# gbordelon/fast_ray_tracer

Hardware: AMD Instinct MI355X
Metric: Mrays/s (primary+shadow+secondary) + wall-clock/frame, 1/2/4/8 GPU (higher is better)
Workload: dtype f64

## Files before the change

### fast_ray_tracer_amd/csrc/frt_engine.hip

```cpp
#include <hip/hip_runtime.h>
#include <hipcub/hipcub.hpp>

#include <algorithm>
#include <array>
#include <atomic>
#include <condition_variable>
#include <memory>
#include <mutex>
#include <cmath>
#include <cstdio>
#include <cstdlib>
#include <cstring>
#include <string>
#include <chrono>
#include <functional>
#include <thread>
#include <vector>

#include "frt_device.h"
#include "frt_jit.h"
#include "frt_shade.hpp"
#include "frt_shade32.hpp"
#include "frt_shadow.hpp"
#include "frt_jit_rt.hpp"
// ... 21 lines not shown
static_assert(sizeof(NodeRec) == 216, "NodeRec layout");

struct NodeCore {
    int32_t material, flags, parent, slot;
    double normalv[3], eyev[3];
    double over_d, rf;
};
struct NodeColors {
    double Ka[3], Kd[3], Ks[3], refl[3];
    double Ns;
};
static_assert(sizeof(NodeCore) == 80 && sizeof(NodeColors) == 104, "NodeCols layout");
enum NodeFlags : int32_t { kReflApplies = 1, kRefrApplies = 2, kMix = 4, kDissolve = 8, kReflSpawned = 16, kRefrSpawned = 32 };
enum : int32_t { kOwnColors = 64, kOwnD = 128 };

struct NodeCols {
    Cols<NodeCore> core;
    Cols<NodeColors> col;
    HeadCols head;
    int32_t root = 0;
    int32_t eye_cam = 0;
    static size_t bytes(int64_t cap) { return Cols<NodeCore>::bytes(cap) + Cols<NodeColors>::bytes(cap); }
    void set(uint64_t* base, int64_t cap) {
        core.w = base;
        core.cap = cap;
        col.w = base + (size_t)Cols<NodeCore>::kWords * cap;
        col.cap = cap;
    }
    __device__ __forceinline__ void store(int64_t i, const NodeRec& v, bool own_colors, bool own_d) const {
        NodeCore c;
        for (int k = 0; k < 3; ++k) {
            c.normalv[k] = v.normalv[k];
            c.eyev[k] = v.eyev[k];
        }
        c.material = v.material;
        c.parent = v.parent;
        c.slot = v.slot;
        c.flags = v.flags | (own_colors ? kOwnColors : 0) | (own_d ? kOwnD : 0);
        c.over_d = v.over_d;
        c.rf = v.rf;
        uint64_t t[10];
        __builtin_memcpy(t, &c, sizeof(c));
        const int64_t cap = core.cap;
        core.w[i] = t[0];
        if (!root) core.w[cap + i] = t[1];
#pragma unroll
        for (int f = 2; f < 5; ++f) core.w[f * cap + i] = t[f];
        if (!eye_cam) {
#pragma unroll
            for (int f = 5; f < 8; ++f) core.w[f * cap + i] = t[f];
        }
        if (own_d) core.w[8 * cap + i] = t[8];
        if (c.flags & kMix) core.w[9 * cap + i] = t[9];
        if (own_colors) {
            NodeColors o;
            for (int k = 0; k < 3; ++k) {
                o.Ka[k] = v.Ka[k];
                o.Kd[k] = v.Kd[k];
                o.Ks[k] = v.Ks[k];
                o.refl[k] = v.refl[k];
            }
            o.Ns = v.Ns;
            col.store(i, o);
        }
    }
    __device__ __forceinline__ void store_miss(int64_t i, int32_t parent, int32_t slot) const {
        core.w[i] = (uint64_t)(uint32_t)-1;
        if (!root) core.w[core.cap + i] = (uint64_t)(uint32_t)parent | ((uint64_t)(uint32_t)slot << 32);
    }
    __device__ __forceinline__ NodeRec load(int64_t i, const frt_material* __restrict__ mats) const {
        uint64_t t[10];
        const int64_t cap = core.cap;
        t[0] = core.w[i];
        t[1] = root ? (uint64_t)(uint32_t)-1 : core.w[cap + i];
#pragma unroll
        for (int f = 2; f < 5; ++f) t[f] = core.w[f * cap + i];
#pragma unroll
        for (int f = 5; f < 8; ++f) t[f] = eye_cam ? 0ull : core.w[f * cap + i];
        const int32_t mat = (int32_t)(uint32_t)t[0], fl = (int32_t)(t[0] >> 32);
        const double od = (fl & kOwnD) ? __longlong_as_double((long long)core.w[8 * cap + i])
                          : mat >= 0 ? 1.0 - mats[mat].Tr : 0.0;
        const double rf = (fl & kMix) ? __longlong_as_double((long long)core.w[9 * cap + i]) : 0.0;
        t[8] = (uint64_t)__double_as_longlong(od);
        t[9] = (uint64_t)__double_as_longlong(rf);
        NodeCore c;
        __builtin_memcpy(&c, t, sizeof(c));
        NodeRec v;
        head.over_point(i, v.over_point);
        for (int k = 0; k < 3; ++k) {
            v.normalv[k] = c.normalv[k];
            v.eyev[k] = c.eyev[k];
        }
        v.key = head.key != nullptr ? head.key[i] : 0ull;
        v.material = c.material;
        v.parent = c.parent;
        v.slot = c.slot;
        v.flags = c.flags;
        v.over_d = c.over_d;
        v.rf = c.rf;
        if (c.material < 0) {
            for (int k = 0; k < 3; ++k) v.Ka[k] = v.Kd[k] = v.Ks[k] = v.refl[k] = 0.0;
            v.Ns = 0.0;
        } else if (c.flags & kOwnColors) {
// ... 380 lines not shown
#define FRT_SHADE_FACTOR 1
#endif
#ifndef FRT_SHADE_ALG
#define FRT_SHADE_ALG 1
#endif
#ifndef FRT_SHADE_SKIP
#define FRT_SHADE_SKIP 1
#endif
#ifndef FRT_SHADE_FMA
#define FRT_SHADE_FMA 1
#endif
__device__ __forceinline__ double dot3_shade(const double* a, const double* b) {
    if (FRT_SHADE_FMA) return __builtin_fma(a[0], b[0], __builtin_fma(a[1], b[1], a[2] * b[2]));
    return dot3(a, b);
}
__device__ __forceinline__ void camera_eyev(const DevScene& S, const Batch& B, int64_t i, double* eyev) {
    Ray r;
    uint64_t key;
    unsigned ce = 0;
    camera_ray(S, B, i, r, key, ce);
    for (int k = 0; k < 3; ++k) eyev[k] = r.d[k] * -1.0;
}

__global__ void __launch_bounds__(kBlock) k_view_rays(DevScene S, Batch B, const frt_camera* __restrict__ cams,
                                                      int32_t nviews, int64_t view_pixels, int64_t n,
                                                      QueuedRay* __restrict__ q, unsigned* err) {
    const int64_t i = (int64_t)blockIdx.x * blockDim.x + threadIdx.x;
    if (i >= n) return;
    const int64_t pix = B.pixel_begin + i / B.spp;
    const int view = (int)min((int64_t)(nviews - 1), pix / view_pixels);
    Batch Bv = B;
    Bv.pixel_begin = pix - (int64_t)view * view_pixels - i / B.spp;
    unsigned e = 0;
    auto emit = [&](const frt_camera& cam) {
        DevScene Sv = S;
        Sv.cam = cam;
// ... 396 lines not shown
        }
    for (int k = 0; k < 3; ++k) {
        out[k] = sA[k];
        out[4 + k] = 0.0;
        out[8 + k] = 0.0;
    }
    out[3] = out[7] = out[11] = 0.0;
}

constexpr int kShadeSegs = 64;
static_assert(kShadeSegs == jit::kMixSegs, "k_shade_lit reads its slots with jit::mix_slot");
template <bool kLazy>
__global__ void __launch_bounds__(kBlock) k_shade(DevScene S, Batch B, NodeCols rec, int64_t n,
                                                  const int32_t* __restrict__ counts, Cols<Tri9> surface,
                                                  uint32_t* __restrict__ lit, unsigned* __restrict__ lcount,
                                                  uint32_t segcap) {
    const int64_t i = (int64_t)blockIdx.x * blockDim.x + threadIdx.x;
    bool heavy = false, mine = false;
    NodeRec nr{};
    if (i < n) {
        nr = rec.load(i, S.materials);
        if (!kLazy) nr.key = rec.key(S, B, i);
        mine = nr.material >= 0;
        heavy = mine && lit != nullptr && shade_heavy(S, counts, i);
    }
    if (!kLazy && mine && !heavy) {
        double out[12];
        if (rec.eye_cam) camera_eyev(S, B, i, nr.eyev);
        shade_node(S, B, nr, i, counts, out);
        tri_store(surface, i, out);
    }
    if (lit != nullptr) {
        const unsigned long long m = __ballot(heavy);
        if (m) {
            const int lane = threadIdx.x & 63;
            const int seg = (int)(blockIdx.x % kShadeSegs);
            unsigned base = 0;
            if (lane == 0) base = atomicAdd(lcount + seg * jit::kMixLine, (unsigned)__popcll(m));
            base = __shfl(base, 0, 64);
            const unsigned at = base + (unsigned)__popcll(m & ((1ull << lane) - 1));
            if (heavy) lit[(size_t)seg * segcap + at] = (uint32_t)i;
        }
    }
// ... 56 lines not shown
    nodes[m] = i;
}

struct LitStage {
    double over_point[3], normalv[3], eyev[3];
    uint64_t key;
    int32_t material, flags;
    uint32_t node;
    int32_t c0;
};
static_assert(sizeof(LitStage) == 96, "LitStage layout");

__global__ void __launch_bounds__(kBlock) k_lit_stage(DevScene S, Batch B, NodeCols rec, const int32_t* __restrict__ counts,
                                                      const uint32_t* __restrict__ lit, const unsigned* __restrict__ lcount,
                                                      uint32_t segcap, int sort_light, uint32_t* __restrict__ rows,
                                                      uint32_t* __restrict__ vals, LitStage* __restrict__ stage) {
    const uint32_t m = blockIdx.x * blockDim.x + threadIdx.x;
    const unsigned total = lit_total(lcount);
    if (blockIdx.x * blockDim.x + (threadIdx.x & ~63u) >= total) return;
    const size_t slot = jit::mix_slot(m < total ? m : 0u, lcount, segcap);
    if (m >= total) return;
    const uint32_t i = lit[slot];
    NodeRec nr = rec.load(i, S.materials);
    nr.key = rec.key(S, B, i);
    if (rec.eye_cam) camera_eyev(S, B, i, nr.eyev);
    LitStage r;
    for (int k = 0; k < 3; ++k) {
        r.over_point[k] = nr.over_point[k];
        r.normalv[k] = nr.normalv[k];
        r.eyev[k] = nr.eyev[k];
    }
    r.key = nr.key;
    r.material = nr.material;
    r.flags = nr.flags;
    r.node = i;
    r.c0 = S.num_lights == 1 ? counts[i] : -1;
    uint64_t w[12];
    __builtin_memcpy(w, &r, sizeof(r));
    uint64_t* dst = (uint64_t*)(stage + m);
#pragma unroll
    for (int k = 0; k < 12; ++k) dst[k] = w[k];
    rows[m] = (uint32_t)light_row(S.lights[sort_light], B.seed, nr.key, sort_light, 1);
    vals[m] = m;
}

#ifndef FRT_SHADE_WAVES
#define FRT_SHADE_WAVES 4
#endif
template <bool kRows, bool kFast32>
__device__ __forceinline__ void shade_lit_body(const DevScene& S, const Batch& B, const NodeCols& rec,
                                               const int32_t* __restrict__ counts, Cols<Tri9> surface,
                                               const uint32_t* __restrict__ lit,
                                               const unsigned* __restrict__ lcount, uint32_t segcap,
                                               const uint32_t* __restrict__ flat,
                                               const LitStage* __restrict__ stage, uint32_t* __restrict__ spos,
                                               const Light32& F) {
    const uint32_t m = blockIdx.x * blockDim.x + threadIdx.x;
    const int lane = threadIdx.x & 63;
    const unsigned c = lcount[lane * jit::kMixLine];
    unsigned incl = c;
#pragma unroll
    for (int o = 1; o < 64; o <<= 1) {
        const unsigned t = __shfl_up(incl, o, 64);
        if (lane >= o) incl += t;
    }
    const unsigned total = __shfl(incl, 63, 64);
    if (blockIdx.x * blockDim.x + (threadIdx.x & ~63u) >= total) return;
    int64_t i = 0;
    NodeRec nr{};
    int32_t c0 = -1;
    const bool staged = kRows && stage != nullptr;
// ... 15 lines not shown
        nr.material = r.material;
        nr.flags = r.flags;
        c0 = r.c0;
        i = (int64_t)r.node;
    } else {
        if (flat != nullptr) {
            if (m >= total) return;
            i = (int64_t)flat[m];
        } else {
            const size_t slot = jit::mix_slot(m < total ? m : 0u, lcount, segcap);
            if (m >= total) return;
            i = (int64_t)lit[slot];
        }
        nr = rec.load(i, S.materials);
        nr.key = rec.key(S, B, i);
        if (rec.eye_cam) camera_eyev(S, B, i, nr.eyev);
    }
    if (staged) {
        if (nr.flags & kOwnColors) {
            const NodeColors o = rec.col.load(i);
            for (int k = 0; k < 3; ++k) {
                nr.Ka[k] = o.Ka[k];
                nr.Kd[k] = o.Kd[k];
                nr.Ks[k] = o.Ks[k];
            }
            nr.Ns = o.Ns;
        } else {
            const frt_material& M = S.materials[nr.material];
            for (int k = 0; k < 3; ++k) {
                nr.Ka[k] = M.Ka[k];
                nr.Kd[k] = M.Kd[k];
// ... 22 lines not shown
            dst[3 + k] = (uint64_t)__double_as_longlong(out[4 + k]);
            dst[6 + k] = (uint64_t)__double_as_longlong(out[8 + k]);
        }
        spos[i] = m;
        return;
    }
    tri_store(surface, i, out);
}

template <bool kRows>
__global__ void __launch_bounds__(kBlock) __attribute__((amdgpu_waves_per_eu(FRT_SHADE_WAVES, 8))) k_shade_lit(DevScene S, Batch B, NodeCols rec,
                                                      const int32_t* __restrict__ counts, Cols<Tri9> surface,
                                                      const uint32_t* __restrict__ lit,
                                                      const unsigned* __restrict__ lcount, uint32_t segcap,
                                                      const uint32_t* __restrict__ flat,
                                                      const LitStage* __restrict__ stage, uint32_t* __restrict__ spos) {
    shade_lit_body<kRows, false>(S, B, rec, counts, surface, lit, lcount, segcap, flat, stage, spos, Light32{});
}

template <bool kRows>
__global__ void __launch_bounds__(kBlock) k_shade_lit32(DevScene S, Batch B, NodeCols rec,
                                                        const int32_t* __restrict__ counts, Cols<Tri9> surface,
                                                        const uint32_t* __restrict__ lit,
                                                        const unsigned* __restrict__ lcount, uint32_t segcap,
                                                        const uint32_t* __restrict__ flat,
                                                        const LitStage* __restrict__ stage, uint32_t* __restrict__ spos,
                                                        Light32 F) {
    shade_lit_body<kRows, true>(S, B, rec, counts, surface, lit, lcount, segcap, flat, stage, spos, F);
}

__device__ __forceinline__ void combine_node(const DevScene& S, const int32_t* __restrict__ counts,
                                             const NodeRec& nr, int64_t i, Cols<Tri9> surface, Cols<Tri9> child,
                                             const frt_material* __restrict__ mats, int32_t include_specular,
                                             double* col, const uint32_t* __restrict__ spos = nullptr) {
    if (nr.material < 0) {
        for (int k = 0; k < 12; ++k) col[k] = 0.0;
        return;
    }
    if (counts != nullptr && !shade_heavy(S, counts, i)) {
        ambient_node(S, nr, col);
    } else if (spos != nullptr) {
        const uint64_t* src = surface.w + (size_t)9 * spos[i];
#pragma unroll
// ... 817 lines not shown
        bool sorted = false;
        int64_t cap = 0;
    };
    std::vector<Level> levels;
    frt::HitRec* hits = nullptr;
    int64_t hits_cap = 0;
    double* hn12 = nullptr;
    int64_t hn12_cap = 0;
    frt::Cols<frt::Tri9> sample_col;
    int64_t sample_cap = 0;
    double* out_dev = nullptr;
    int64_t out_cap = 0;
    frt_camera* view_cams = nullptr;
    int64_t view_cams_cap = 0;
    int32_t strip_views = 0;
    frt::QueuedRay* view_q = nullptr;
    int64_t view_q_cap = 0;
    unsigned long long* counters = nullptr;
    unsigned* err = nullptr;
    hipEvent_t ev[2] = {nullptr, nullptr};
    struct Mark {
        int slot;
        size_t a, b;
    };
    std::vector<hipEvent_t> ev_pool;
    std::vector<Mark> ev_marks;
    size_t ev_used = 0;
    std::vector<frt_light> host_lights;
    struct Gi {
        bool built = false;
// ... 1121 lines not shown
                (void)hipGetLastError();
                frt_scene_release(h);
                return fail("frt_scene_upload: " + std::to_string(h->lds_bytes) +
                            " B of LDS per traversal block refused (" + hipGetErrorString(e) + ")");
            }
        }
    }
    {
        const char* wf = std::getenv("FRT_WALK_FLAGS");
        S.walk_flags = wf ? std::atoi(wf) : 0;
    }
    S.num_nodes = sc->num_nodes;
    S.num_roots = sc->num_roots;
    S.num_lights = sc->num_lights;
    S.num_patterns = sc->num_patterns;
    S.cam = sc->camera;
    S.cfg = sc->config;
    h->host_lights.assign(sc->lights, sc->lights + sc->num_lights);
    {
        const char* e = std::getenv("FRT_SHADE_SORT");
        h->sort_light = -1;
        for (int l = 0; l < sc->num_lights && h->sort_light < 0 && !(e && std::atoi(e) == 0); ++l)
            if (sc->lights[l].rows > 1 && sc->lights[l].num_samples > 0) h->sort_light = l;
        const char* se = std::getenv("FRT_SHADE_STAGE");
        h->shade_stage = h->sort_light >= 0 ? (se ? std::atoi(se) : 2) : 0;
        const char* qs = std::getenv("FRT_QUEUE_SORT");
        h->queue_sort = qs ? std::atoi(qs) : 2;
        const char* qsh = std::getenv("FRT_QUEUE_SORT_SHIFT");
        h->queue_sort_shift = qsh ? std::max(0, std::min(16, std::atoi(qsh))) : 0;
        const char* pu = std::getenv("FRT_PREPARE_UNIFORM");
// ... 162 lines not shown
    hip_ignore(hipFree(h->tredo));
    hip_ignore(hipFree(h->tbox));
    hip_ignore(hipFree(h->err));
    for (hipEvent_t e : h->ev_pool) hip_ignore(hipEventDestroy(e));
    if (h->ev[0]) hip_ignore(hipEventDestroy(h->ev[0]));
    if (h->ev[1]) hip_ignore(hipEventDestroy(h->ev[1]));
    if (h->stream) hip_ignore(hipStreamDestroy(h->stream));
    delete h;
}

static int32_t level_eye_cam(const frt_scene_handle* h, size_t d) {
    static const bool eye_cam_env = !(std::getenv("FRT_EYE_CAM") && std::atoi(std::getenv("FRT_EYE_CAM")) == 0);
    return d == 0 && !h->S.cfg.use_gi && eye_cam_env && h->strip_views == 0 ? 1 : 0;
}

static bool level_keyed(const frt_scene_handle* h, size_t d) {
    bool multi = false;
    for (const auto& L : h->host_lights) multi = multi || L.rows > 1;
    const char* e = std::getenv("FRT_HEAD_KEY0");
    if (e && std::atoi(e) == 0) multi = false;
    return d > 0 || h->S.cfg.use_gi || h->strip_views > 0 || multi;
}

static int set_level_head(frt_scene_handle* h, size_t d) {
    auto& L = h->levels[d];
    if (L.cap <= 0) return 0;
    if (level_keyed(h, d) && L.head_key == nullptr)
        FRT_HIP(hipMalloc((void**)&L.head_key, (size_t)L.cap * sizeof(uint64_t)));
    L.rec.head.op = L.head_op;
    L.rec.head.key = level_keyed(h, d) ? L.head_key : nullptr;
// ... 17 lines not shown
    hip_ignore(hipFree(L.child.w));
    hip_ignore(hipFree(L.counts));
    hip_ignore(hipFree(L.spos));
    L.spos = nullptr;
    L.rec = {};
    L.q = nullptr;
    L.surface = {};
    L.child = {};
    L.counts = nullptr;
    {
        void* p = nullptr;
        FRT_HIP(hipMalloc(&p, frt::NodeCols::bytes(nc)));
        L.rec.set((uint64_t*)p, nc);
        L.rec.root = d == 0 ? 1 : 0;
        L.rec.eye_cam = level_eye_cam(h, d);
    }
    FRT_HIP(hipMalloc((void**)&L.head_op, (size_t)nc * 3 * sizeof(double)));
    FRT_HIP(hipMalloc((void**)&L.q, nc * sizeof(frt::QueuedRay)));
    FRT_HIP(hipMalloc((void**)&L.surface.w, frt::Cols<frt::Tri9>::bytes(nc)));
    L.surface.cap = nc;
    FRT_HIP(hipMalloc((void**)&L.child.w, frt::Cols<frt::Tri9>::bytes(2 * nc)));
    L.child.cap = 2 * nc;
    if (!L.qprefix) FRT_HIP(hipMalloc((void**)&L.qprefix, (frt::kQueueSegs + 1) * sizeof(int64_t)));
    FRT_HIP(hipMalloc((void**)&L.counts, nc * std::max(1, h->S.num_lights) * sizeof(int32_t)));
    if (h->shade_stage) FRT_HIP(hipMalloc((void**)&L.spos, nc * sizeof(uint32_t)));
    L.cap = nc;
    return set_level_head(h, d);
}

static inline unsigned grid_for(int64_t n, int block = frt::kBlock) { return (unsigned)((n + block - 1) / block); }
// ... 1178 lines not shown
    return rc;
}

static int render_strip(frt_scene_handle* h, const frt_camera* cams, int32_t nviews, const frt_frame_params* P,
                        double* dev_out, frt_frame_stats* st) {
    FRT_HIP(hipSetDevice(h->device));
    if (grow(&h->view_cams, h->view_cams_cap, nviews)) return -1;
    FRT_HIP(hipMemcpy(h->view_cams, cams, (size_t)nviews * sizeof(frt_camera), hipMemcpyHostToDevice));
    const frt_camera own = h->S.cam;
    h->S.cam = cams[0];
    h->strip_views = nviews;
    const int rc = render_impl(h, P, dev_out, st);
    h->strip_views = 0;
    h->S.cam = own;
    if (!h->levels.empty()) h->levels[0].rec.eye_cam = level_eye_cam(h, 0);
    return rc;
}

static int render_frame(frt_scene_handle* h, const frt_frame_params* P, double* dev_out, frt_frame_stats* st) {
    using namespace frt;
    FRT_HIP(hipSetDevice(h->device));
    if (frame_precision(h, P)) return -1;
    if (h->fast32 && ensure_light32(h)) return -1;
    const int64_t hs = h->S.cam.hsize;
    const int64_t stride = P->row_stride > 0 ? P->row_stride : 1;
    int64_t nrows = 0;
    for (int64_t r = P->row_begin; r < P->row_end; r += stride) nrows++;
    const int32_t nviews = h->strip_views;
    const int64_t npix = nrows * hs * std::max(1, nviews);
    if (!h->levels.empty()) h->levels[0].rec.eye_cam = level_eye_cam(h, 0);
    if (!h->levels.empty() && set_level_head(h, 0)) return -1;
    const int32_t spp = (int32_t)(h->S.cam.usteps * h->S.cam.vsteps);
    if (spp <= 0) return fail("render: usteps*vsteps must be positive");
    const char* benv = std::getenv("FRT_BATCH_SAMPLES");
    const int64_t bdef = benv && std::atoll(benv) > 0 ? (int64_t)std::atoll(benv) : (int64_t)1 << 23;
    int64_t batch = P->batch_samples > 0 ? P->batch_samples : bdef;
    int64_t pix_per_batch = std::max<int64_t>(1, batch / spp);
    const int path = h->S.cfg.path_length;
    if (st) {
        std::memset(st, 0, sizeof(*st));
        (void)hipEventRecord(h->ev[0], h->stream);
    }
    FRT_HIP(hipMemsetAsync(h->err, 0, sizeof(unsigned), h->stream));
    FRT_HIP(hipMemsetAsync(h->counters, 0, frt::kQueueSegs * frt::kCounterLine * sizeof(unsigned long long), h->stream));
    if (h->S.cfg.use_gi && (!h->gi.built || h->gi.seed != P->seed)) {
// ... 129 lines not shown
                std::vector<int32_t> hc((size_t)n * h->S.num_lights);
                std::vector<uint64_t> hh((size_t)n);
                FRT_HIP(hipMemcpyAsync(hc.data(), L.counts, hc.size() * sizeof(int32_t), hipMemcpyDeviceToHost, h->stream));
                FRT_HIP(hipMemcpyAsync(hh.data(), L.rec.core.w, hh.size() * sizeof(uint64_t), hipMemcpyDeviceToHost, h->stream));
                FRT_HIP(hipStreamSynchronize(h->stream));
                for (int64_t i = 0; i < n; ++i) {
                    if ((int32_t)(uint32_t)hh[(size_t)i] < 0) continue;
                    for (int l = 0; l < h->S.num_lights; ++l) {
                        const int32_t c = hc[(size_t)(i * h->S.num_lights + l)];
                        h->uniform_stats[c == 0 ? 1 : (c == h->host_lights[(size_t)l].num_samples ? 0 : 2)]++;
                    }
                }
            }
            {
                KTimer t(h, st, 2);
                const bool split = shade_split();
                const int64_t nblocks = grid_for(n);
                const uint32_t segcap = (uint32_t)(((nblocks + kShadeSegs - 1) / kShadeSegs) * kBlock);
                if (split && (grow(&h->shade_lit, h->shade_lit_cap, (int64_t)segcap * kShadeSegs) ||
                              grow(&h->shade_lcount, h->shade_lcount_cap, (int64_t)kShadeSegs * jit::kMixLine)))
                    return -1;
                if (split)
                    FRT_HIP(hipMemsetAsync(h->shade_lcount, 0, (size_t)kShadeSegs * jit::kMixLine * sizeof(unsigned),
                                           h->stream));
                const bool sorted = split && h->sort_light >= 0;
                const int nrows = sorted ? std::max(1, h->host_lights[(size_t)h->sort_light].rows) : 0;
                int row_bits = 1;
                while (row_bits < 32 && (1ll << row_bits) < nrows) ++row_bits;
                const bool sorted_out = sorted && shade_lazy(h) && L.spos != nullptr && h->shade_stage > 0;
                const bool staged = sorted_out && h->shade_stage == 1;
                L.staged = sorted_out;
                if (sorted) {
                    const int64_t lcap = (int64_t)segcap * kShadeSegs;
                    if (grow(&h->lit_row, h->lit_row_cap, 2 * lcap) || grow(&h->lit_flat, h->lit_flat_cap, 2 * lcap))
                        return -1;
                    if (staged && grow(&h->lit_stage, h->lit_stage_cap, lcap)) return -1;
                }
                if (shade_lazy(h))
                    hipLaunchKernelGGL(k_shade<true>, dim3(grid_for(n)), dim3(kBlock), 0, h->stream, h->S, B, L.rec, n,
                                       L.counts, L.surface, h->shade_lit, h->shade_lcount, segcap);
                else
                    hipLaunchKernelGGL(k_shade<false>, dim3(grid_for(n)), dim3(kBlock), 0, h->stream, h->S, B, L.rec, n,
                                       L.counts, L.surface, split ? h->shade_lit : nullptr, h->shade_lcount, segcap);
                if (sorted) {
                    KTimer ts(h, st, 16);
                    const int64_t lcap = (int64_t)segcap * kShadeSegs;
                    uint32_t *keys = h->lit_row, *keys2 = h->lit_row + lcap, *vals = h->lit_flat + lcap;
                    if (staged)
                        hipLaunchKernelGGL(k_lit_stage, dim3(grid_for(n)), dim3(kBlock), 0, h->stream, h->S, B, L.rec,
                                           L.counts, h->shade_lit, h->shade_lcount, segcap, h->sort_light, keys, vals,
                                           h->lit_stage);
                    else
                        hipLaunchKernelGGL(k_lit_rows, dim3(grid_for(n)), dim3(kBlock), 0, h->stream, h->S, B, L.rec.head,
                                           h->shade_lit, h->shade_lcount, segcap, h->sort_light, keys, vals);
                    auto& lc = h->host_lcount;
                    FRT_HIP(hipMemcpyAsync(lc.data(), h->shade_lcount, lc.size() * sizeof(unsigned), hipMemcpyDeviceToHost,
                                           h->stream));
                    FRT_HIP(stream_sync(h));
                    int64_t listed = 0;
                    for (int sgi = 0; sgi < kShadeSegs; ++sgi) listed += lc[(size_t)sgi * jit::kMixLine];
                    if (st != nullptr) st->lit_nodes += (uint64_t)listed;
                    if (listed > 0) {
                        size_t tmp_bytes = 0;
                        FRT_HIP(hipcub::DeviceRadixSort::SortPairs(nullptr, tmp_bytes, keys, keys2, vals, h->lit_flat,
                                                                   (int)listed, 0, row_bits, h->stream));
                        if (grow(&h->scan_tmp, h->scan_tmp_cap, (int64_t)tmp_bytes + 16)) return -1;
// ... 6 lines not shown
                    FRT_HIP(hipMemcpyAsync(lc.data(), h->shade_lcount, lc.size() * sizeof(unsigned), hipMemcpyDeviceToHost,
                                           h->stream));
                    FRT_HIP(hipStreamSynchronize(h->stream));
                    for (int sgi = 0; sgi < kShadeSegs; ++sgi) st->lit_nodes += lc[(size_t)sgi * jit::kMixLine];
                }
#ifndef FRT_SHADE_LIT_BLOCK
#define FRT_SHADE_LIT_BLOCK 64
#endif
                if (split && h->fast32) {
                    KTimer tl(h, st, 17);
                    hipLaunchKernelGGL(sorted ? k_shade_lit32<true> : k_shade_lit32<false>,
                                       dim3(grid_for(n, FRT_SHADE_LIT_BLOCK)), dim3(FRT_SHADE_LIT_BLOCK), 0, h->stream,
                                       h->S, B, L.rec, L.counts, L.surface, h->shade_lit, h->shade_lcount, segcap,
                                       sorted ? (const uint32_t*)h->lit_flat : nullptr,
                                       staged ? (const frt::LitStage*)h->lit_stage : nullptr,
                                       sorted_out ? L.spos : nullptr, h->light32);
                } else if (split) {
                    KTimer tl(h, st, 15);
                    hipLaunchKernelGGL(sorted ? k_shade_lit<true> : k_shade_lit<false>, dim3(grid_for(n, FRT_SHADE_LIT_BLOCK)),
                                       dim3(FRT_SHADE_LIT_BLOCK), 0,
                                       h->stream, h->S, B, L.rec, L.counts, L.surface, h->shade_lit, h->shade_lcount, segcap,
                                       sorted ? (const uint32_t*)h->lit_flat : nullptr,
                                       staged ? (const frt::LitStage*)h->lit_stage : nullptr,
                                       sorted_out ? L.spos : nullptr);
                }
                FRT_HIP(hipGetLastError());
            }
            if (h->S.cfg.use_gi) {
                KTimer t(h, st, 7);
                if (shade_gi(h, B, L, n, st)) return -1;
            }
            if (h->sync_epoch == counters_epoch) FRT_HIP(stream_sync(h));
            int64_t next = 0;
            bool overflow = false;
            for (int j = 0; j < kQueueSegs && !dense; ++j) {
                N.hprefix[j] = next;
                int64_t c = (int64_t)host_counters[(size_t)j * kCounterLine + d + 1];
                if (c > B.next_segcap) {
                    overflow = true;
// ... 69 lines not shown
            hipLaunchKernelGGL(k_resolve, dim3((unsigned)((bp + 63) / 64)), dim3(kResolveBlock), 0, h->stream, h->sample_col, bp, spp,
                               dev_out + 4 * p0);
            FRT_HIP(hipGetLastError());
        }
    }
    FRT_HIP(hipMemcpyAsync(host_counters.data(), h->counters, host_counters.size() * sizeof(unsigned long long),
                           hipMemcpyDeviceToHost, h->stream));
    unsigned err = 0;
    FRT_HIP(hipMemcpyAsync(&err, h->err, sizeof(unsigned), hipMemcpyDeviceToHost, h->stream));
    if (st) (void)hipEventRecord(h->ev[1], h->stream);
    FRT_HIP(hipStreamSynchronize(h->stream));
    if (st) {
        float ms = 0.f;
        (void)hipEventElapsedTime(&ms, h->ev[0], h->ev[1]);
        st->render_ms = ms;
        uint64_t pruned = 0, hits = 0, uniform_waves = 0;
        for (int j = 0; j < kQueueSegs; ++j) {
            pruned += host_counters[(size_t)j * kCounterLine + 16];
            hits += host_counters[(size_t)j * kCounterLine + 17];
            uniform_waves += host_counters[(size_t)j * kCounterLine + 18];
        }
        st->prepare_uniform_waves = uniform_waves;
        st->pruned_secondary = pruned;
        st->hits = hits;
        st->shadow_rays = h->S.cfg.include_direct ? hits * (uint64_t)h->samples_per_node : 0;
        bool multi = false;
        for (const auto& L : h->host_lights) multi = multi || L.rows > 1;
        const double kHead = multi ? 40.0 : 32.0;
        st->shadow_kernel_bytes = !(h->S.cfg.include_direct && h->samples_per_node > 0) ? 0.0
                                  : h->jit_shadow != nullptr ? (double)h->pairs_walked * 8.0 + (double)h->heads_walked * (kHead + 4.0) +
                                                                   (multi ? 24.0 * (double)h->rays_walked : 0.0)
                                                             : (double)hits * (kHead + 4.0 * h->S.num_lights);
        st->errors = err;
        st->shadow_jit = h->jit_shadow != nullptr ? 1 : 0;
        st->shadow_rays_walked = h->jit_shadow != nullptr ? h->rays_walked : st->shadow_rays;
        st->shadow_tile_pairs = h->tile_pairs;
        st->shadow_tile_mixed = h->tile_mixed;
// ... 179 lines not shown
```

### fast_ray_tracer_amd/csrc/frt_shade.hpp

```cpp
#pragma once

#include "frt_traverse.hpp"

namespace frt {

template <class T>
__device__ __forceinline__ const T* const_table(const T* p) {
    return (const T*)(const __attribute__((address_space(4))) T*)(uint64_t)p;
}
__device__ __forceinline__ DevScene uniform_view(const DevScene& S) {
    DevScene U = S;
    U.nodes = const_table(S.nodes);
    U.xchain = const_table(S.xchain);
    U.xforms = const_table(S.xforms);
    U.prim = const_table(S.prim);
    U.materials = const_table(S.materials);
    return U;
}

__device__ __forceinline__ int first_xf(const DevScene& S, int leaf) {
    return S.nodes[leaf].xform >= 0 ? leaf : S.nodes[leaf].tparent;
}

__device__ inline void world_to_object(const DevScene& S, int leaf, const double* p, double* out, bool w0 = false) {
// ... 431 lines not shown
    local_normal(S, leaf, lp, h, ln);
    normal_to_world(S, leaf, ln);
    const frt_material& M = S.materials[S.nodes[leaf].material];
    if (kPat && M.map_bump >= 0) {
        double tmp[3];
        pattern_at_shape<kPatternDepth>(S, M.map_bump, leaf, wp, tmp);
        for (int k = 0; k < 3; ++k) {
            tmp[k] *= 2.0;
            ln[k] += tmp[k] - 1.0;
        }
    }
    normalize3(ln, n);
}

template <bool kPat = true>
__device__ inline void prepare(const DevScene& S, const Ray& r, Hit h, Comps& c) {
    if (S.nodes[h.node].type == FRT_TRIANGLE || S.nodes[h.node].type == FRT_SMOOTH_TRIANGLE) {
        LeafHits H;
        const Ray lr = leaf_local_ray(S, h.node, r);
        leaf_hits<false>(S.nodes[h.node].type, S.prim + S.nodes[h.node].prim, lr, H);
        if (H.t.n > 0) {
            h.u = H.u;
            h.v = H.v;
        }
    }
    c.leaf = h.node;
    c.material = S.nodes[h.node].material;
    for (int k = 0; k < 3; ++k) c.p[k] = r.o[k] + r.d[k] * h.t;
    normal_at<kPat>(S, h.node, c.p, h, c.normalv);
    for (int k = 0; k < 3; ++k) c.eyev[k] = r.d[k] * -1.0;
    if (dot3(c.normalv, c.eyev) < 0) {
        for (int k = 0; k < 3; ++k) c.normalv[k] *= -1;
    }
    double dd = 2 * dot3(r.d, c.normalv);
    for (int k = 0; k < 3; ++k) c.reflectv[k] = r.d[k] - c.normalv[k] * dd;
    for (int k = 0; k < 3; ++k) {
        c.over_point[k] = c.p[k] + c.normalv[k] * kEps;
        c.under_point[k] = c.p[k] - c.normalv[k] * kEps;
    }
    c.n1 = 1.0;
    c.n2 = 1.0;
    const frt_material& M = S.materials[c.material];
    if (kPat && M.map_Ka >= 0) pattern_at_shape<kPatternDepth>(S, M.map_Ka, c.leaf, c.over_point, c.Ka);
    else copy3(M.Ka, c.Ka);
    if (kPat && M.map_Kd >= 0) pattern_at_shape<kPatternDepth>(S, M.map_Kd, c.leaf, c.over_point, c.Kd);
    else copy3(M.Kd, c.Kd);
    if (kPat && M.map_Ks >= 0) pattern_at_shape<kPatternDepth>(S, M.map_Ks, c.leaf, c.over_point, c.Ks);
    else copy3(M.Ks, c.Ks);
// ... 33 lines not shown
```

### fast_ray_tracer_amd/runtime.py

```python
from __future__ import annotations

import ctypes
import os
import weakref
import threading

import numpy as np

from . import build

_lock = threading.Lock()
_host = None


class FrameParams(ctypes.Structure):
    _fields_ = [("row_begin", ctypes.c_int64), ("row_end", ctypes.c_int64), ("row_stride", ctypes.c_int64),
                ("seed", ctypes.c_uint64), ("batch_samples", ctypes.c_int64),
                ("count_reference_rays", ctypes.c_int32), ("precision", ctypes.c_int32)]


PRECISION = {None: 0, "parity": 1, "fast32": 2}


class FrameStats(ctypes.Structure):
    _fields_ = [("primary_rays", ctypes.c_uint64), ("secondary_rays", ctypes.c_uint64),
                ("shadow_rays", ctypes.c_uint64), ("pruned_secondary", ctypes.c_uint64),
                ("hits", ctypes.c_uint64), ("errors", ctypes.c_uint64), ("render_ms", ctypes.c_double),
                ("kernel_ms", ctypes.c_double * 8), ("kernel_launches", ctypes.c_uint64 * 8),
                ("shadow_kernel_bytes", ctypes.c_double), ("gather_rays", ctypes.c_uint64),
                ("photons", ctypes.c_uint64 * 2), ("photon_ms", ctypes.c_double),
                ("shadow_jit", ctypes.c_int32), ("photon_pass", ctypes.c_int32),
                ("sub_ms", ctypes.c_double * 16), ("sub_launches", ctypes.c_uint64 * 16),
                ("shadow_rays_walked", ctypes.c_uint64), ("shadow_tile_pairs", ctypes.c_uint64),
                ("shadow_tile_mixed", ctypes.c_uint64), ("shadow_pairs", ctypes.c_uint64),
                ("shadow_pairs_mixed", ctypes.c_uint64), ("shadow_sub_pairs", ctypes.c_uint64),
                ("shadow_sub_mixed", ctypes.c_uint64), ("shadow_subtile_pairs", ctypes.c_uint64),
                ("shadow_subtile_mixed", ctypes.c_uint64), ("lit_nodes", ctypes.c_uint64),
                ("prepare_uniform_waves", ctypes.c_uint64)]

    def as_dict(self) -> dict:
        names = ["trace", "shadow", "shade", "combine", "resolve", "trace_primary", "prepare", "gi"]
        subs = ["frt_jit_beam", "frt_jit_shadow", "k_gather_est", "k_gather_hit", "frt_jit_tile", "frt_jit_sub",
                "frt_jit_subtile", "k_shade_lit", "k_lit_sort", "k_shade_lit32"]
        return {
            "primary_rays": int(self.primary_rays), "secondary_rays": int(self.secondary_rays),
            "shadow_rays": int(self.shadow_rays), "pruned_secondary": int(self.pruned_secondary),
            "hits": int(self.hits), "errors": int(self.errors), "render_ms": float(self.render_ms),
            "shadow_kernel_bytes": float(self.shadow_kernel_bytes),
            "gather_rays": int(self.gather_rays), "photons": [int(self.photons[0]), int(self.photons[1])],
            "photon_ms": float(self.photon_ms), "shadow_jit": int(self.shadow_jit),
            "photon_pass": int(self.photon_pass),
            "kernel_ms": {names[i]: float(self.kernel_ms[i]) for i in range(8) if self.kernel_launches[i]},
            "kernel_launches": {names[i]: int(self.kernel_launches[i]) for i in range(8) if self.kernel_launches[i]},
            "sub_ms": {subs[i]: float(self.sub_ms[i]) for i in range(len(subs)) if self.sub_launches[i]},
            "sub_launches": {subs[i]: int(self.sub_launches[i]) for i in range(len(subs)) if self.sub_launches[i]},
            "shadow_rays_walked": int(self.shadow_rays_walked),
            "shadow_tile_pairs": int(self.shadow_tile_pairs), "shadow_tile_mixed": int(self.shadow_tile_mixed),
            "shadow_pairs": int(self.shadow_pairs), "shadow_pairs_mixed": int(self.shadow_pairs_mixed),
            "shadow_sub_pairs": int(self.shadow_sub_pairs), "shadow_sub_mixed": int(self.shadow_sub_mixed),
            "shadow_subtile_pairs": int(self.shadow_subtile_pairs),
            "shadow_subtile_mixed": int(self.shadow_subtile_mixed), "lit_nodes": int(self.lit_nodes),
            "prepare_uniform_waves": int(self.prepare_uniform_waves),
        }


class EncodeStats(ctypes.Structure):
    _fields_ = [("values", ctypes.c_uint64), ("undecided", ctypes.c_uint64), ("backend", ctypes.c_int32),
                ("decline", ctypes.c_int32), ("mode", ctypes.c_int32), ("device", ctypes.c_int32),
                ("rgb_max", ctypes.c_double * 3), ("srgb_max", ctypes.c_double * 3), ("upload_ms", ctypes.c_double),
                ("kernel_ms", ctypes.c_double), ("readback_ms", ctypes.c_double), ("patch_ms", ctypes.c_double),
                ("host_ms", ctypes.c_double)]

    def as_dict(self) -> dict:
        return {"values": int(self.values), "undecided": int(self.undecided),
                "backend": ENCODE_BACKENDS[self.backend], "decline": ENCODE_DECLINES[self.decline],
                "mode": ENCODE_MODES[self.mode], "device": int(self.device), "rgb_max": list(self.rgb_max),
                "srgb_max": list(self.srgb_max), "upload_ms": float(self.upload_ms),
# ... 511 lines not shown
```

### include/frt_device.h

```cpp
#ifndef FRT_DEVICE_H
#define FRT_DEVICE_H

#ifndef __HIPCC_RTC__
#include <stddef.h>
#include <stdint.h>
#endif

#ifdef __cplusplus
extern "C" {
#endif

#define FRT_ABI_VERSION 3u

enum frt_node_type {
    FRT_CONE = 0,
    FRT_CUBE = 1,
    FRT_CYLINDER = 2,
    FRT_PLANE = 3,
    FRT_SMOOTH_TRIANGLE = 4,
    FRT_SPHERE = 5,
    FRT_TOROID = 6,
    FRT_TRIANGLE = 7,
    FRT_CSG = 8,
    FRT_GROUP = 9
// ... 152 lines not shown
    int32_t shadow_jit;
    int32_t photon_pass;
    double sub_ms[16];
    uint64_t sub_launches[16];
    uint64_t shadow_rays_walked;
    uint64_t shadow_tile_pairs;
    uint64_t shadow_tile_mixed;
    uint64_t shadow_pairs;
    uint64_t shadow_pairs_mixed;
    uint64_t shadow_sub_pairs;
    uint64_t shadow_sub_mixed;
    uint64_t shadow_subtile_pairs;
    uint64_t shadow_subtile_mixed;
    uint64_t lit_nodes;
    uint64_t prepare_uniform_waves;
} frt_frame_stats;

int frt_device_count(void);

int frt_device_warmup(int device);

void *frt_host_pinned_alloc(size_t bytes);
void frt_host_pinned_free(void *p);

size_t frt_frame_stats_size(void);

size_t frt_frame_params_size(void);

const char *frt_last_error(void);

// ... 89 lines not shown
```

Measured before the change: 521,000.

## Recompute level-0 normals and over points in shading instead of storing them

```diff
diff --git a/fast_ray_tracer_amd/csrc/frt_engine.hip b/fast_ray_tracer_amd/csrc/frt_engine.hip
--- a/fast_ray_tracer_amd/csrc/frt_engine.hip
+++ b/fast_ray_tracer_amd/csrc/frt_engine.hip
@@ -59,12 +59,17 @@
 enum NodeFlags : int32_t { kReflApplies = 1, kRefrApplies = 2, kMix = 4, kDissolve = 8, kReflSpawned = 16, kRefrSpawned = 32 };
 enum : int32_t { kOwnColors = 64, kOwnD = 128 };
 
+#ifndef FRT_NORM_OVER
+#define FRT_NORM_OVER 1
+#endif
+
 struct NodeCols {
     Cols<NodeCore> core;
     Cols<NodeColors> col;
     HeadCols head;
     int32_t root = 0;
     int32_t eye_cam = 0;
+    int32_t norm_cam = 0;
     static size_t bytes(int64_t cap) { return Cols<NodeCore>::bytes(cap) + Cols<NodeColors>::bytes(cap); }
     void set(uint64_t* base, int64_t cap) {
         core.w = base;
@@ -89,8 +94,10 @@
         const int64_t cap = core.cap;
         core.w[i] = t[0];
         if (!root) core.w[cap + i] = t[1];
+        if (!norm_cam) {
 #pragma unroll
-        for (int f = 2; f < 5; ++f) core.w[f * cap + i] = t[f];
+            for (int f = 2; f < 5; ++f) core.w[f * cap + i] = t[f];
+        }
         if (!eye_cam) {
 #pragma unroll
             for (int f = 5; f < 8; ++f) core.w[f * cap + i] = t[f];
@@ -119,7 +126,7 @@
         t[0] = core.w[i];
         t[1] = root ? (uint64_t)(uint32_t)-1 : core.w[cap + i];
 #pragma unroll
-        for (int f = 2; f < 5; ++f) t[f] = core.w[f * cap + i];
+        for (int f = 2; f < 5; ++f) t[f] = norm_cam ? 0ull : core.w[f * cap + i];
 #pragma unroll
         for (int f = 5; f < 8; ++f) t[f] = eye_cam ? 0ull : core.w[f * cap + i];
         const int32_t mat = (int32_t)(uint32_t)t[0], fl = (int32_t)(t[0] >> 32);
@@ -131,7 +138,8 @@
         NodeCore c;
         __builtin_memcpy(&c, t, sizeof(c));
         NodeRec v;
-        head.over_point(i, v.over_point);
+        if (FRT_NORM_OVER && norm_cam) v.over_point[0] = v.over_point[1] = v.over_point[2] = 0.0;
+        else head.over_point(i, v.over_point);
         for (int k = 0; k < 3; ++k) {
             v.normalv[k] = c.normalv[k];
             v.eyev[k] = c.eyev[k];
@@ -542,12 +550,38 @@
     if (FRT_SHADE_FMA) return __builtin_fma(a[0], b[0], __builtin_fma(a[1], b[1], a[2] * b[2]));
     return dot3(a, b);
 }
-__device__ __forceinline__ void camera_eyev(const DevScene& S, const Batch& B, int64_t i, double* eyev) {
+struct NormSrc {
+    const HitRec* hits;
+    unsigned long long* counters;
+    int32_t uniform_ok;
+};
+template <bool kCount>
+__device__ __forceinline__ void derive_node(const DevScene& S, const Batch& B, const NodeCols& rec, const NormSrc& src,
+                                            int64_t i, NodeRec& nr) {
+    if (!rec.eye_cam && !rec.norm_cam) return;
     Ray r;
     uint64_t key;
     unsigned ce = 0;
     camera_ray(S, B, i, r, key, ce);
-    for (int k = 0; k < 3; ++k) eyev[k] = r.d[k] * -1.0;
+    if (rec.eye_cam)
+        for (int k = 0; k < 3; ++k) nr.eyev[k] = r.d[k] * -1.0;
+    if (!rec.norm_cam) return;
+    const HitRec hr = src.hits[i];
+    double p[3];
+    auto normal = [&](const DevScene& S, const int leaf) __attribute__((always_inline)) {
+        hit_normal<false>(S, r, Hit{hr.t, -1, -1, leaf}, p, nr.normalv);
+    };
+    const int leaf_u = uniform(hr.node);
+    if (src.uniform_ok && __ballot(hr.node != leaf_u) == 0ull) {
+        if (kCount && B.stats)
+            wave_count(src.counters + kCounterLine * (blockIdx.x % kQueueSegs) + 19,
+                       (int)(threadIdx.x & 63) == __builtin_ctzll(__ballot(true)));
+        normal(uniform_view(S), leaf_u);
+    } else {
+        normal(S, hr.node);
+    }
+    if (FRT_NORM_OVER)
+        for (int k = 0; k < 3; ++k) nr.over_point[k] = p[k] + nr.normalv[k] * kEps;
 }
 
 __global__ void __launch_bounds__(kBlock) k_view_rays(DevScene S, Batch B, const frt_camera* __restrict__ cams,
@@ -974,7 +1008,7 @@
 __global__ void __launch_bounds__(kBlock) k_shade(DevScene S, Batch B, NodeCols rec, int64_t n,
                                                   const int32_t* __restrict__ counts, Cols<Tri9> surface,
                                                   uint32_t* __restrict__ lit, unsigned* __restrict__ lcount,
-                                                  uint32_t segcap) {
+                                                  uint32_t segcap, NormSrc src) {
     const int64_t i = (int64_t)blockIdx.x * blockDim.x + threadIdx.x;
     bool heavy = false, mine = false;
     NodeRec nr{};
@@ -986,7 +1020,7 @@
     }
     if (!kLazy && mine && !heavy) {
         double out[12];
-        if (rec.eye_cam) camera_eyev(S, B, i, nr.eyev);
+        derive_node<false>(S, B, rec, src, i, nr);
         shade_node(S, B, nr, i, counts, out);
         tri_store(surface, i, out);
     }
@@ -1073,7 +1107,8 @@
 __global__ void __launch_bounds__(kBlock) k_lit_stage(DevScene S, Batch B, NodeCols rec, const int32_t* __restrict__ counts,
                                                       const uint32_t* __restrict__ lit, const unsigned* __restrict__ lcount,
                                                       uint32_t segcap, int sort_light, uint32_t* __restrict__ rows,
-                                                      uint32_t* __restrict__ vals, LitStage* __restrict__ stage) {
+                                                      uint32_t* __restrict__ vals, LitStage* __restrict__ stage,
+                                                      NormSrc src) {
     const uint32_t m = blockIdx.x * blockDim.x + threadIdx.x;
     const unsigned total = lit_total(lcount);
     if (blockIdx.x * blockDim.x + (threadIdx.x & ~63u) >= total) return;
@@ -1082,7 +1117,7 @@
     const uint32_t i = lit[slot];
     NodeRec nr = rec.load(i, S.materials);
     nr.key = rec.key(S, B, i);
-    if (rec.eye_cam) camera_eyev(S, B, i, nr.eyev);
+    derive_node<true>(S, B, rec, src, i, nr);
     LitStage r;
     for (int k = 0; k < 3; ++k) {
         r.over_point[k] = nr.over_point[k];
@@ -1113,7 +1148,7 @@
                                                const unsigned* __restrict__ lcount, uint32_t segcap,
                                                const uint32_t* __restrict__ flat,
                                                const LitStage* __restrict__ stage, uint32_t* __restrict__ spos,
-                                               const Light32& F) {
+                                               const NormSrc& src, const Light32& F) {
     const uint32_t m = blockIdx.x * blockDim.x + threadIdx.x;
     const int lane = threadIdx.x & 63;
     const unsigned c = lcount[lane * jit::kMixLine];
@@ -1159,7 +1194,7 @@
         }
         nr = rec.load(i, S.materials);
         nr.key = rec.key(S, B, i);
-        if (rec.eye_cam) camera_eyev(S, B, i, nr.eyev);
+        derive_node<true>(S, B, rec, src, i, nr);
     }
     if (staged) {
         if (nr.flags & kOwnColors) {
@@ -1212,8 +1247,9 @@
                                                       const uint32_t* __restrict__ lit,
                                                       const unsigned* __restrict__ lcount, uint32_t segcap,
                                                       const uint32_t* __restrict__ flat,
-                                                      const LitStage* __restrict__ stage, uint32_t* __restrict__ spos) {
-    shade_lit_body<kRows, false>(S, B, rec, counts, surface, lit, lcount, segcap, flat, stage, spos, Light32{});
+                                                      const LitStage* __restrict__ stage, uint32_t* __restrict__ spos,
+                                                      NormSrc src) {
+    shade_lit_body<kRows, false>(S, B, rec, counts, surface, lit, lcount, segcap, flat, stage, spos, src, Light32{});
 }
 
 template <bool kRows>
@@ -1223,8 +1259,8 @@
                                                         const unsigned* __restrict__ lcount, uint32_t segcap,
                                                         const uint32_t* __restrict__ flat,
                                                         const LitStage* __restrict__ stage, uint32_t* __restrict__ spos,
-                                                        Light32 F) {
-    shade_lit_body<kRows, true>(S, B, rec, counts, surface, lit, lcount, segcap, flat, stage, spos, F);
+                                                        NormSrc src, Light32 F) {
+    shade_lit_body<kRows, true>(S, B, rec, counts, surface, lit, lcount, segcap, flat, stage, spos, src, F);
 }
 
 __device__ __forceinline__ void combine_node(const DevScene& S, const int32_t* __restrict__ counts,
@@ -2072,6 +2108,7 @@
     frt_camera* view_cams = nullptr;
     int64_t view_cams_cap = 0;
     int32_t strip_views = 0;
+    bool bump_maps = false;
     frt::QueuedRay* view_q = nullptr;
     int64_t view_q_cap = 0;
     unsigned long long* counters = nullptr;
@@ -3223,6 +3260,8 @@
     S.num_roots = sc->num_roots;
     S.num_lights = sc->num_lights;
     S.num_patterns = sc->num_patterns;
+    h->bump_maps = false;
+    for (int32_t m = 0; m < sc->num_materials; ++m) h->bump_maps = h->bump_maps || sc->materials[m].map_bump >= 0;
     S.cam = sc->camera;
     S.cfg = sc->config;
     h->host_lights.assign(sc->lights, sc->lights + sc->num_lights);
@@ -3415,6 +3454,12 @@
     return d == 0 && !h->S.cfg.use_gi && eye_cam_env && h->strip_views == 0 ? 1 : 0;
 }
 
+static int32_t level_norm_cam(const frt_scene_handle* h, size_t d) {
+    const char* e = std::getenv("FRT_NORMAL0");
+    const bool norm_env = !(e && std::atoi(e) == 0);
+    return d == 0 && !h->S.cfg.use_gi && h->strip_views == 0 && !h->bump_maps && norm_env ? 1 : 0;
+}
+
 static bool level_keyed(const frt_scene_handle* h, size_t d) {
     bool multi = false;
     for (const auto& L : h->host_lights) multi = multi || L.rows > 1;
@@ -3462,6 +3507,7 @@
         L.rec.set((uint64_t*)p, nc);
         L.rec.root = d == 0 ? 1 : 0;
         L.rec.eye_cam = level_eye_cam(h, d);
+        L.rec.norm_cam = level_norm_cam(h, d);
     }
     FRT_HIP(hipMalloc((void**)&L.head_op, (size_t)nc * 3 * sizeof(double)));
     FRT_HIP(hipMalloc((void**)&L.q, nc * sizeof(frt::QueuedRay)));
@@ -4670,6 +4716,7 @@
     h->strip_views = 0;
     h->S.cam = own;
     if (!h->levels.empty()) h->levels[0].rec.eye_cam = level_eye_cam(h, 0);
+    if (!h->levels.empty()) h->levels[0].rec.norm_cam = level_norm_cam(h, 0);
     return rc;
 }
 
@@ -4685,6 +4732,7 @@
     const int32_t nviews = h->strip_views;
     const int64_t npix = nrows * hs * std::max(1, nviews);
     if (!h->levels.empty()) h->levels[0].rec.eye_cam = level_eye_cam(h, 0);
+    if (!h->levels.empty()) h->levels[0].rec.norm_cam = level_norm_cam(h, 0);
     if (!h->levels.empty() && set_level_head(h, 0)) return -1;
     const int32_t spp = (int32_t)(h->S.cam.usteps * h->S.cam.vsteps);
     if (spp <= 0) return fail("render: usteps*vsteps must be positive");
@@ -4844,6 +4892,7 @@
             }
             {
                 KTimer t(h, st, 2);
+                const NormSrc nsrc{h->hits, h->counters, h->prepare_uniform};
                 const bool split = shade_split();
                 const int64_t nblocks = grid_for(n);
                 const uint32_t segcap = (uint32_t)(((nblocks + kShadeSegs - 1) / kShadeSegs) * kBlock);
@@ -4868,10 +4917,10 @@
                 }
                 if (shade_lazy(h))
                     hipLaunchKernelGGL(k_shade<true>, dim3(grid_for(n)), dim3(kBlock), 0, h->stream, h->S, B, L.rec, n,
-                                       L.counts, L.surface, h->shade_lit, h->shade_lcount, segcap);
+                                       L.counts, L.surface, h->shade_lit, h->shade_lcount, segcap, nsrc);
                 else
                     hipLaunchKernelGGL(k_shade<false>, dim3(grid_for(n)), dim3(kBlock), 0, h->stream, h->S, B, L.rec, n,
-                                       L.counts, L.surface, split ? h->shade_lit : nullptr, h->shade_lcount, segcap);
+                                       L.counts, L.surface, split ? h->shade_lit : nullptr, h->shade_lcount, segcap, nsrc);
                 if (sorted) {
                     KTimer ts(h, st, 16);
                     const int64_t lcap = (int64_t)segcap * kShadeSegs;
@@ -4879,7 +4928,7 @@
                     if (staged)
                         hipLaunchKernelGGL(k_lit_stage, dim3(grid_for(n)), dim3(kBlock), 0, h->stream, h->S, B, L.rec,
                                            L.counts, h->shade_lit, h->shade_lcount, segcap, h->sort_light, keys, vals,
-                                           h->lit_stage);
+                                           h->lit_stage, nsrc);
                     else
                         hipLaunchKernelGGL(k_lit_rows, dim3(grid_for(n)), dim3(kBlock), 0, h->stream, h->S, B, L.rec.head,
                                            h->shade_lit, h->shade_lcount, segcap, h->sort_light, keys, vals);
@@ -4916,7 +4965,7 @@
                                        h->S, B, L.rec, L.counts, L.surface, h->shade_lit, h->shade_lcount, segcap,
                                        sorted ? (const uint32_t*)h->lit_flat : nullptr,
                                        staged ? (const frt::LitStage*)h->lit_stage : nullptr,
-                                       sorted_out ? L.spos : nullptr, h->light32);
+                                       sorted_out ? L.spos : nullptr, nsrc, h->light32);
                 } else if (split) {
                     KTimer tl(h, st, 15);
                     hipLaunchKernelGGL(sorted ? k_shade_lit<true> : k_shade_lit<false>, dim3(grid_for(n, FRT_SHADE_LIT_BLOCK)),
@@ -4924,7 +4973,7 @@
                                        h->stream, h->S, B, L.rec, L.counts, L.surface, h->shade_lit, h->shade_lcount, segcap,
                                        sorted ? (const uint32_t*)h->lit_flat : nullptr,
                                        staged ? (const frt::LitStage*)h->lit_stage : nullptr,
-                                       sorted_out ? L.spos : nullptr);
+                                       sorted_out ? L.spos : nullptr, nsrc);
                 }
                 FRT_HIP(hipGetLastError());
             }
@@ -5024,13 +5073,16 @@
         float ms = 0.f;
         (void)hipEventElapsedTime(&ms, h->ev[0], h->ev[1]);
         st->render_ms = ms;
-        uint64_t pruned = 0, hits = 0, uniform_waves = 0;
+        uint64_t pruned = 0, hits = 0, uniform_waves = 0, shade_uniform = 0;
         for (int j = 0; j < kQueueSegs; ++j) {
             pruned += host_counters[(size_t)j * kCounterLine + 16];
             hits += host_counters[(size_t)j * kCounterLine + 17];
             uniform_waves += host_counters[(size_t)j * kCounterLine + 18];
+            shade_uniform += host_counters[(size_t)j * kCounterLine + 19];
         }
         st->prepare_uniform_waves = uniform_waves;
+        st->level0_normals_derived = !h->levels.empty() && h->levels[0].rec.norm_cam ? 1 : 0;
+        st->shade_uniform_waves = shade_uniform;
         st->pruned_secondary = pruned;
         st->hits = hits;
         st->shadow_rays = h->S.cfg.include_direct ? hits * (uint64_t)h->samples_per_node : 0;
diff --git a/fast_ray_tracer_amd/csrc/frt_shade.hpp b/fast_ray_tracer_amd/csrc/frt_shade.hpp
--- a/fast_ray_tracer_amd/csrc/frt_shade.hpp
+++ b/fast_ray_tracer_amd/csrc/frt_shade.hpp
@@ -469,7 +469,7 @@
 }
 
 template <bool kPat = true>
-__device__ inline void prepare(const DevScene& S, const Ray& r, Hit h, Comps& c) {
+__device__ inline void hit_normal(const DevScene& S, const Ray& r, Hit h, double* p, double* normalv) {
     if (S.nodes[h.node].type == FRT_TRIANGLE || S.nodes[h.node].type == FRT_SMOOTH_TRIANGLE) {
         LeafHits H;
         const Ray lr = leaf_local_ray(S, h.node, r);
@@ -479,14 +479,21 @@
             h.v = H.v;
         }
     }
+    for (int k = 0; k < 3; ++k) p[k] = r.o[k] + r.d[k] * h.t;
+    normal_at<kPat>(S, h.node, p, h, normalv);
+    double eyev[3];
+    for (int k = 0; k < 3; ++k) eyev[k] = r.d[k] * -1.0;
+    if (dot3(normalv, eyev) < 0) {
+        for (int k = 0; k < 3; ++k) normalv[k] *= -1;
+    }
+}
+
+template <bool kPat = true>
+__device__ inline void prepare(const DevScene& S, const Ray& r, Hit h, Comps& c) {
     c.leaf = h.node;
     c.material = S.nodes[h.node].material;
-    for (int k = 0; k < 3; ++k) c.p[k] = r.o[k] + r.d[k] * h.t;
-    normal_at<kPat>(S, h.node, c.p, h, c.normalv);
+    hit_normal<kPat>(S, r, h, c.p, c.normalv);
     for (int k = 0; k < 3; ++k) c.eyev[k] = r.d[k] * -1.0;
-    if (dot3(c.normalv, c.eyev) < 0) {
-        for (int k = 0; k < 3; ++k) c.normalv[k] *= -1;
-    }
     double dd = 2 * dot3(r.d, c.normalv);
     for (int k = 0; k < 3; ++k) c.reflectv[k] = r.d[k] - c.normalv[k] * dd;
     for (int k = 0; k < 3; ++k) {
diff --git a/fast_ray_tracer_amd/runtime.py b/fast_ray_tracer_amd/runtime.py
--- a/fast_ray_tracer_amd/runtime.py
+++ b/fast_ray_tracer_amd/runtime.py
@@ -36,7 +36,8 @@
                 ("shadow_pairs_mixed", ctypes.c_uint64), ("shadow_sub_pairs", ctypes.c_uint64),
                 ("shadow_sub_mixed", ctypes.c_uint64), ("shadow_subtile_pairs", ctypes.c_uint64),
                 ("shadow_subtile_mixed", ctypes.c_uint64), ("lit_nodes", ctypes.c_uint64),
-                ("prepare_uniform_waves", ctypes.c_uint64)]
+                ("prepare_uniform_waves", ctypes.c_uint64), ("level0_normals_derived", ctypes.c_uint64),
+                ("shade_uniform_waves", ctypes.c_uint64)]
 
     def as_dict(self) -> dict:
         names = ["trace", "shadow", "shade", "combine", "resolve", "trace_primary", "prepare", "gi"]
@@ -61,6 +62,8 @@
             "shadow_subtile_pairs": int(self.shadow_subtile_pairs),
             "shadow_subtile_mixed": int(self.shadow_subtile_mixed), "lit_nodes": int(self.lit_nodes),
             "prepare_uniform_waves": int(self.prepare_uniform_waves),
+            "level0_normals_derived": int(self.level0_normals_derived),
+            "shade_uniform_waves": int(self.shade_uniform_waves),
         }
 
 
diff --git a/include/frt_device.h b/include/frt_device.h
--- a/include/frt_device.h
+++ b/include/frt_device.h
@@ -190,6 +190,8 @@
     uint64_t shadow_subtile_mixed;
     uint64_t lit_nodes;
     uint64_t prepare_uniform_waves;
+    uint64_t level0_normals_derived;
+    uint64_t shade_uniform_waves;
 } frt_frame_stats;
 
 int frt_device_count(void);
```

New measurement: 522,500, median of 6. No clear change (+0.3%).
